# jnhansen/nd

Measured on AMD Instinct MI355X. Metric: Mpixels/s OmnibusTest dual-pol 24t x 4096 x 4096, higher is better.
Workload: dtype f32; 1 GPU; OmnibusTest C2 24t x 4096 x 4096 f32 per GPU (BASELINE configs[1]), resident in HBM; looks=9, rows_per_rank=4096

## Files before the change

### nd_amd/csrc/omnibus.hip

```cpp
#include <type_traits>

#include "omnibus_c2_device.hpp"

namespace nd_amd {

template <typename T, int PPT, bool STATS>
__global__ void __launch_bounds__(kGlobalThreads)
omnibus_c2_global_kernel(const OmniGlobalArgs<T> g, const OmniTab tab)
{
    const int tid = threadIdx.x;
    const int lane = tid & 63;
    const int64_t b = blockIdx.x;
    const int64_t row = b / g.blocks_per_row;
    const int64_t bx = b - row * g.blocks_per_row;
    const int64_t bpx0 = bx * (int64_t)(kGlobalThreads * PPT);
    const int64_t x0 = bpx0 + (int64_t)tid * PPT;
    const int k = g.k;

    if (g.write_tab && b == 0) {
        for (int j = tid; j <= k; j += kGlobalThreads) g.tab_dev[j] = tab.e[j];
    }

    {
        int64_t npx = g.nx - bpx0;
// ... 982 lines not shown
    uint32_t segd;
    const OmniTabEntry *tab;
    uint32_t *flag_idx;
    uint32_t seg;
    T *dump;
    uint32_t dump_cap;
};



__device__ __forceinline__ void store_change_row(uint8_t *res, const int k, const unsigned long long mask)
{
    if ((k & 3) == 0 && ((uintptr_t)res & 3) == 0) {
        uint32_t *w = reinterpret_cast<uint32_t *>(res);
        for (int q = 0; q < (k >> 2); ++q) {
            const unsigned nib = (unsigned)(mask >> (4 * q)) & 0xFu;
            w[q] = (nib * 0x00204081u) & 0x01010101u;
        }
    } else {
        for (int t = 0; t < k; ++t) res[t] = (uint8_t)((mask >> t) & 1ull);
    }
}

template <typename T, int KMAX>
__global__ void __launch_bounds__(64, 2) omnibus_c2_dense_kernel(const OmniDenseArgs<T> s,
                                                              const StreamScreen<32> ss)
{
    __shared__ StreamEntry tab_lds[33];
    const int lane = threadIdx.x;
    const unsigned shard = blockIdx.x % kShards;
    const unsigned lblock = blockIdx.x / kShards, nlblock = gridDim.x / kShards;
    const uint32_t n = s.flag_count[shard * kCounterStride + 1];
    if (lblock >= n) return;
    const uint32_t *list = s.dense_idx + (size_t)shard * s.segd;
    if (lane <= 32) tab_lds[lane] = ss.e[lane];
    __syncthreads();

    for (uint32_t w = lblock; w < n; w += nlblock) {
        int k = s.k;
        asm volatile("" : "+s"(k));
        const int64_t pix0 = (int64_t)(uint32_t)__builtin_amdgcn_readfirstlane((int)list[w]);
        const int64_t pix = pix0 + lane;
        const int64_t row0 = pix0 / s.nx;
        const int64_t col0 = pix0 - row0 * s.nx;
        int64_t ub;
        unsigned delta;
        bool active;
        if (s.flat) {
            active = pix < s.npix;
            ub = pix0;
            delta = (unsigned)((active ? pix : s.npix - 1) - pix0);
        } else {
            active = col0 + lane < s.nx;
            ub = row0 * s.sy + col0 * s.sx;
            delta = (unsigned)(((active ? col0 + lane : s.nx - 1) - col0) * s.sx);
        }
        T v[KMAX][4];
#pragma unroll
        for (int t = 0; t < KMAX; ++t) {
            const int64_t ot = ub + (int64_t)(t < k ? t : k - 1) * s.st;
            v[t][0] = (s.c11 + ot)[delta];
            v[t][1] = (s.c12r + ot)[delta];
            v[t][2] = (s.c12i + ot)[delta];
            v[t][3] = (s.c22 + ot)[delta];
        }
        __builtin_amdgcn_sched_barrier(0);
        unsigned mask;
        bool handoff, cand;
        dense_chain<T, KMAX, 32>(v, k, active, ss, tab_lds, mask, handoff, cand);
        if (active && !handoff && mask != 0u) store_change_row(s.change + pix * (int64_t)k, k, mask);
        if (__any(handoff)) {
            const unsigned long long m = __ballot(handoff);
            unsigned base = 0;
            if (lane == 0) base = atomicAdd(s.flag_count + shard * kCounterStride, (unsigned)__popcll(m));
            base = __shfl(base, 0);
            if (handoff) {
                const unsigned slot = base + (unsigned)__popcll(m & ((1ull << lane) - 1ull));
                s.flag_idx[(size_t)shard * s.seg + slot] = (uint32_t)pix;
                if (slot < s.dump_cap) {
                    T *d = s.dump + ((int64_t)shard * s.dump_cap + slot) * (int64_t)(4 * k);
#pragma unroll
                    for (int t = 0; t < KMAX; ++t)
                        if (t < k) {
                            Pack<T, 4> q;
                            q.v[0] = v[t][0];
                            q.v[1] = v[t][1];
                            q.v[2] = v[t][2];
                            q.v[3] = v[t][3];
// ... 1001 lines not shown
                    o.v[3] = q.d;
                    *reinterpret_cast<Pack<T, 4> *>(d + 4 * t) = o;
                }
            }
        }
    }
    if (!dense && wnp > 0) zero_fill_span(wob, wnp * k, lane);
}

template <typename T>
struct OmniSearchArgs {
    const T *c11, *c12r, *c12i, *c22;
    int64_t nx;
    int64_t sy, sx, st;
    int m11, m12, m22;
    int k;
    double nlooks, alpha;
    uint8_t *change;
    const uint32_t *flag_count, *flag_idx;
    uint32_t seg;
    const OmniTabEntry *tab;
    const T *dump;
    uint32_t dump_cap;
    unsigned long long *hand_bits;
    uint32_t hand_words;
    uint32_t *hand_count;
    uint32_t starts_max;
    uint32_t first;
};

constexpr int kScreenLong = 192;
struct DenseScreenLong {
    DenseScreenEntry e[kScreenLong + 1];
};

template <typename T, int MODE, int PXW = 64, bool FS = false, bool GSCR = false>
__global__ void __launch_bounds__(64) omnibus_c2_search_kernel(const OmniSearchArgs<T> s, const DenseScreenLong fscr)
{
    static_assert(!GSCR || (MODE == 1 && !FS), "the global-memory screen serves the double screen of MODE 1");
    constexpr bool USE_LDS = (MODE == 0);
    extern __shared__ __align__(16) unsigned char nd_smem[];
    T *lds = reinterpret_cast<T *>(nd_smem);
    const int lane = threadIdx.x;
    const int k = s.k;
    const OmniTabEntry *tabp = s.tab;
    const int kp = k + 1;
    double *scr = reinterpret_cast<double *>(nd_smem + (USE_LDS ? (size_t)k * 4 * PXW * sizeof(T) : 0));
    DenseScreenEntry *scr_f = reinterpret_cast<DenseScreenEntry *>(scr);
    if (FS) {
// ... 2 lines not shown
    } else if (!GSCR) {
        for (int j = lane; j <= k; j += 64) {
            const OmniTabEntry e = s.tab[j];
            scr[j] = e.m2rho;
            scr[kp + j] = e.pklogk;
            scr[2 * kp + j] = e.zlo_a;
            scr[3 * kp + j] = e.zhi_a;
        }
        __syncthreads();
    }
    auto screen = [&](int f, int j) -> double {
        if (GSCR) return f == 0 ? tabp[j].m2rho : (f == 1 ? tabp[j].pklogk : (f == 2 ? tabp[j].zlo_a : tabp[j].zhi_a));
        return scr[f * kp + j];
    };
    const unsigned shard = blockIdx.x % kShards;
    const unsigned lblock = blockIdx.x / kShards;
    const unsigned nlblock = gridDim.x / kShards;
    const uint32_t n = s.flag_count[shard * kCounterStride];
    const uint32_t *list = s.flag_idx + (size_t)shard * s.seg;
    if (n <= s.starts_max) return;

    for (uint32_t base = s.first + lblock * (unsigned)PXW; base < n; base += nlblock * (unsigned)PXW) {
        const uint32_t idx = base + lane;
        bool active = idx < n && lane < PXW;
        if (s.hand_bits != nullptr) {
            if (__builtin_nontemporal_load(s.hand_count) == 0u) return;
            const unsigned long long marked = s.hand_bits[(size_t)shard * s.hand_words + (base >> 6)];
            if (marked == 0ull) continue;
            active = active && ((marked >> lane) & 1ull);
        }
        const int64_t pix = active ? (int64_t)list[idx] : 0;
        const int64_t row = pix / s.nx;
        const int64_t col = pix - row * s.nx;
        const int64_t off = row * s.sy + col * s.sx;

        if (USE_LDS && (PXW == 64 || lane < PXW)) {
            if (idx < s.dump_cap) {
                const T *d = s.dump + ((int64_t)shard * s.dump_cap + idx) * (int64_t)(4 * k);
                for (int t0 = 0; t0 < k; t0 += 8) {
                    Pack<T, 4> q[8];
#pragma unroll
                    for (int u = 0; u < 8; ++u)
                        if (t0 + u < k)
                            q[u] = *reinterpret_cast<const Pack<T, 4> *>(d + 4 * (t0 + u));
#pragma unroll
                    for (int u = 0; u < 8; ++u)
                        if (t0 + u < k) {
                            const int t = t0 + u;
                            lds[(t * 4 + 0) * PXW + lane] = q[u].v[0];
                            lds[(t * 4 + 1) * PXW + lane] = q[u].v[1];
                            lds[(t * 4 + 2) * PXW + lane] = q[u].v[2];
                            lds[(t * 4 + 3) * PXW + lane] = q[u].v[3];
                        }
// ... 214 lines not shown
                        }
                    }
                }
            }
            if (!done) {
                if (fires && (k - l) >= 2) {
                    res[fire_at] = 1;
                    l = fire_at;
                    if (l >= k - 1) {
                        done = true;
                    } else {
                        A.reset();
                        fire_at = -1;
                    }
                } else {
                    done = true;
                }
            }
        }
    }
}

template <typename T>
__global__ void __launch_bounds__(64) omnibus_c2_search_starts_kernel(const OmniSearchArgs<T> s)
{
    const int lane = threadIdx.x;
    const int k = s.k;
    const int ns = k - 1;
    const int ppw = ns <= 64 ? 64 / ns : 1;
    const int nsw = ns <= 64 ? ns : 64;
    const int nsweep = ns <= 64 ? 1 : (ns <= 128 ? 2 : 3);
    const int grp = lane / nsw;
    const int l0 = lane - grp * nsw;
    const unsigned shard = blockIdx.x % kShards;
    const unsigned lblock = blockIdx.x / kShards;
    const unsigned nlblock = gridDim.x / kShards;
    const uint32_t n = s.flag_count[shard * kCounterStride];
    const bool marked_mode = s.hand_bits != nullptr;
    if (marked_mode ? (n <= s.starts_max) : (n > s.starts_max)) return;
    if (marked_mode && __builtin_nontemporal_load(s.hand_count) == 0u) return;
    const uint32_t *list = s.flag_idx + (size_t)shard * s.seg;
    const OmniTabEntry *tabp = s.tab;

    uint32_t word = lblock;
    unsigned long long todo = 0ull;
    for (uint32_t base = lblock * (uint32_t)ppw;; base += nlblock * (uint32_t)ppw) {
        uint32_t idx;
        bool active;
        if (marked_mode) {
            while (todo == 0ull && (uint64_t)word * 64u < n) {
                todo = s.hand_bits[(size_t)shard * s.hand_words + word];
                if (todo == 0ull) word += nlblock;
            }
            if (todo == 0ull) break;
            unsigned long long m = todo;
            for (int i = 0; i < grp; ++i) m &= m - 1ull;
            active = (grp < ppw) && (m != 0ull);
            idx = word * 64u + (uint32_t)(m != 0ull ? __builtin_ctzll(m) : 0);
            for (int i = 0; i < ppw; ++i) todo &= todo - 1ull;
            if (todo == 0ull) word += nlblock;
        } else {
            if (base >= n) break;
            idx = base + (uint32_t)grp;
            active = (grp < ppw) && (idx < n);
        }
        const int64_t pix = active ? (int64_t)list[idx] : 0;
        const int64_t row = pix / s.nx;
        const int64_t col = pix - row * s.nx;
        const int64_t off = row * s.sy + col * s.sx;
        const bool from_dump = active && idx < s.dump_cap;
        const T *dsrc = s.dump + ((int64_t)shard * s.dump_cap + (from_dump ? idx : 0)) * (int64_t)(4 * k);
        auto fetch = [&](int t) -> Pack<T, 4> {
            Pack<T, 4> q;
            if (from_dump) {
                q = *reinterpret_cast<const Pack<T, 4> *>(dsrc + 4 * t);
            } else {
                const int64_t o = off + (int64_t)t * s.st;
                q.v[0] = s.c11[o * s.m11];
                q.v[1] = s.c12r[o * s.m12];
                q.v[2] = s.c12i[o * s.m12];
                q.v[3] = s.c22[o * s.m22];
            }
            return q;
        };
        int nxt_a = -1, nxt_b = -1, nxt_c = -1;
        for (int sweep = 0; sweep < nsweep; ++sweep) {
        const int l = l0 + 64 * sweep;
        const bool lact = active && l < ns;
        Accum<T> A;
        A.reset();
        int fire_at = -1;
        int nxt = -1;
        auto fetch4 = [&](const int i0, Pack<T, 4> (&q)[4]) {
#pragma unroll
            for (int u = 0; u < 4; ++u) {
                const int t = l + i0 + u;
                q[u].v[0] = q[u].v[1] = q[u].v[2] = q[u].v[3] = (T)0;
                if (lact && t < k) q[u] = fetch(t);
            }
        };
        Pack<T, 4> qn[4];
        fetch4(0, qn);
        for (int i0 = 0; i0 < k; i0 += 4) {
            if (!__any(lact && l + i0 < k)) break;
            Pack<T, 4> q[4];
#pragma unroll
            for (int u = 0; u < 4; ++u) q[u] = qn[u];
            fetch4(i0 + 4, qn);
#pragma unroll
            for (int u = 0; u < 4; ++u) {
                const int i = i0 + u;
                const int t = l + i;
                const bool on = lact && t < k;
                if (on) A.step(q[u].v[0], q[u].v[1], q[u].v[2], q[u].v[3]);
                const int jj = i + 1;
                const bool last = (t == k - 1);
                const bool need = on && (jj >= 2) && (fire_at < 0 || last);
                bool fires = false, inband = false;
                if (need) {
                    const OmniTabEntry &e = tabp[jj];
                    const double za = z_approx<T>(A, jj, s.nlooks, e.m2rho, e.pklogk);
                    fires = (za > e.zhi_a) && (za < INFINITY);
                    inband = (za >= e.zlo_a) && !fires;
                }
                if (__any(inband)) {
                    if (inband) {
                        const OmniTabEntry e = tabp[jj];
                        const T zp = z_stat<T>(A, jj, s.nlooks, e);
                        const double zd = (double)zp;
                        int verdict = !(zd >= e.zlo) ? 0 : ((zd > e.zhi && zd < INFINITY) ? 1 : 2);
                        if (verdict == 2) {
                            double zv[1] = {zd}, P1[1], P2[1];
                            chisq_pair<1>(zv, 4 * (jj - 1), e.lgam, P1, P2);
                            const T P = combine_P<T>(P1[0], P2[0], e.omega2);
                            verdict = ((double)P > s.alpha) ? 1 : 0;
                        }
                        fires = (verdict == 1);
                    }
                }
                if (on && fires && fire_at < 0) fire_at = t;
                if (on && last && fires) nxt = fire_at;
            }
        }
        if (sweep == 0) nxt_a = nxt; else if (sweep == 1) nxt_b = nxt; else nxt_c = nxt;
        }
        int at = 0;
        for (int step = 0; step < ns; ++step) {
            const int ats = (at >= 0 && at < ns) ? at : 0;
            const int src = grp * nsw + (ats & 63) % nsw;
            const int na = __shfl(nxt_a, src), nb = __shfl(nxt_b, src), nc = __shfl(nxt_c, src);
            const int n1 = (ns > 64 && ats >= 128) ? nc : ((ns > 64 && ats >= 64) ? nb : na);
            if (at >= 0 && at < ns) {
                if (n1 < 0) {
                    at = -1;
                } else {
                    if (active && l0 == 0) s.change[pix * (int64_t)k + n1] = 1;
                    at = n1;
                }
            }
        }
    }
}

template <typename T, int KMAX>
__global__ void __launch_bounds__(64, 3)
omnibus_c2_search_chain_kernel(const OmniSearchArgs<T> s, const StreamScreen<32> ss)
{
    __shared__ StreamEntry tab_lds[33];
    const int lane = threadIdx.x;
    if (lane <= 32) tab_lds[lane] = ss.e[lane];
    __syncthreads();
    int k = s.k;
    asm volatile("" : "+s"(k));
    const unsigned shard = blockIdx.x % kShards;
    const unsigned lblock = blockIdx.x / kShards;
    const unsigned nlblock = gridDim.x / kShards;
    const uint32_t n = s.flag_count[shard * kCounterStride];
    if (n <= s.starts_max) return;
    const uint32_t *list = s.flag_idx + (size_t)shard * s.seg;

    for (uint32_t base = lblock * 64u; base < n; base += nlblock * 64u) {
        const uint32_t idx = base + lane;
        const bool active = idx < n;
        const int64_t pix = active ? (int64_t)list[idx] : 0;
        T v[KMAX][4];
        if (idx < s.dump_cap) {
            const T *d = s.dump + ((int64_t)shard * s.dump_cap + idx) * (int64_t)(4 * k);
#pragma unroll
            for (int t = 0; t < KMAX; ++t) {
                const Pack<T, 4> q = *reinterpret_cast<const Pack<T, 4> *>(d + 4 * (t < k ? t : k - 1));
                v[t][0] = q.v[0];
                v[t][1] = q.v[1];
                v[t][2] = q.v[2];
                v[t][3] = q.v[3];
            }
        } else {
            const int64_t row = pix / s.nx;
            const int64_t col = pix - row * s.nx;
            const int64_t off = row * s.sy + col * s.sx;
            const T *p11 = s.c11 + off * s.m11, *p12r = s.c12r + off * s.m12;
            const T *p12i = s.c12i + off * s.m12, *p22 = s.c22 + off * s.m22;
            const int64_t d11 = s.st * s.m11, d12 = s.st * s.m12, d22 = s.st * s.m22;
#pragma unroll
            for (int t = 0; t < KMAX; ++t) {
                v[t][0] = *p11;
                v[t][1] = *p12r;
                v[t][2] = *p12i;
                v[t][3] = *p22;
                if (t < k - 1) {
                    p11 += d11;
                    p12r += d12;
                    p12i += d12;
                    p22 += d22;
                }
            }
        }
        unsigned cmask;
        bool handoff, cand;
        dense_chain<T, KMAX, 32>(v, k, active, ss, tab_lds, cmask, handoff, cand);
        {
            const unsigned long long hm = __ballot(handoff);
            if (lane == 0) {
                s.hand_bits[(size_t)shard * s.hand_words + (base >> 6)] = hm;
                if (hm != 0ull) atomicAdd(s.hand_count, (unsigned)__popcll(hm));
            }
        }
        if (active && !handoff) {
            uint8_t *res = s.change + pix * (int64_t)k;
            for (int u = 1; u < k; ++u)
                if ((cmask >> u) & 1u) res[u] = 1;
        }
    }
}

std::vector<OmniTabEntry> get_table_impl(int k, uint32_t n_looks, double alpha, int dtype, int pol)
{
    static std::mutex mu;
    static std::vector<TabCacheEntry> cache;
    {
        std::lock_guard<std::mutex> lk(mu);
        for (const auto &c : cache)
            if (c.key.k == k && c.key.dtype == dtype && c.key.pol == pol && c.key.n == n_looks &&
                memcmp(&c.key.alpha, &alpha, sizeof(double)) == 0)
                return c.tab;
    }
    std::vector<OmniTabEntry> tab((size_t)k + 1);
    memset(tab.data(), 0, tab.size() * sizeof(OmniTabEntry));
    for (int j = 1; j <= k; ++j)
        tab[j] = dtype == ND_AMD_F32 ? make_entry<float>(j, n_looks, alpha, pol)
                                     : make_entry<double>(j, n_looks, alpha, pol);
    {
        std::lock_guard<std::mutex> lk(mu);
        if (cache.size() >= 32) cache.erase(cache.begin());
// ... 241 lines not shown
                          k <= (sizeof(T) == 4 ? 192 : 96) && pm_ids == nullptr && mlp == nullptr && sx == 1;
    static const bool gate_env = env_int("ND_AMD_GATE", 1) != 0;
    g.gate = flag_count + 2;
    g.gate_n = 0;
    g.gate_mode = 0;
    {
        const size_t per = (size_t)k * 4 * sizeof(T);
        size_t cap = (retain || stream_long || split_ok) ? (workspace_bytes - w.off_dump) / per / kShards : 0;
        g.seg = w.seg;
        if (cap > g.seg) cap = g.seg;
        if (split_ok) cap &= ~(size_t)63;
        g.dump = reinterpret_cast<T *>(ws + w.off_dump);
        g.dump_cap = (uint32_t)cap;
    }

    constexpr int VPPT = 16 / sizeof(T);
    const size_t es = sizeof(T);
    const bool aligned = (sx == 1) && (((uintptr_t)c11 | (uintptr_t)c12re | (uintptr_t)c12im |
                                        (uintptr_t)c22) & 15) == 0 &&
                         ((sy * (int64_t)es) % 16 == 0) && ((st * (int64_t)es) % 16 == 0);
    const bool flat = ((sx == 1) && (sy == nx)) || pm_ids != nullptr;
    g.nx = flat ? npix : nx;
    g.nrows = flat ? 1 : ny;
    unsigned long long *const hand_ws = reinterpret_cast<unsigned long long *>(ws + w.off_hand);
    const int ppt = retain ? 1 : (aligned ? VPPT : 1);
    g.blocks_per_row = ceil_div(g.nx, retain ? (int64_t)kRetainThreads : (int64_t)kGlobalThreads * ppt);
    const int64_t nblocks = g.blocks_per_row * g.nrows;
    if (nblocks > 0x7fffffffLL) {
        set_error("nd_amd_omnibus_c2: raster too large for one launch (%lld blocks)",
                  (long long)nblocks);
        return ND_AMD_EUNSUPPORTED;
    }
    auto take_sample = [&]() -> bool {
        const int64_t sblocks_total = ceil_div(npix, (int64_t)kRetainThreads);
        if (!gate_env || !retain || sblocks_total < 4096) return false;
        OmniSampleArgs<T> sa;
        sa.c11 = g.c11;
        sa.c12r = g.c12r;
        sa.c12i = g.c12i;
        sa.c22 = g.c22;
        sa.nx = g.nx;
        sa.blocks_per_row = ceil_div(g.nx, (int64_t)kRetainThreads);
        const int64_t total = sa.blocks_per_row * g.nrows;
        const int64_t nsb = pm_ids ? 128 : 512;
        sa.block_stride = total / nsb;
        sa.sy = sy;
        sa.sx = sx;
// ... 34 lines not shown
        d.tab = tab_dev;
        d.flag_idx = idx;
        d.seg = seg;
        d.dump = dump;
        d.dump_cap = dump_cap;
        int64_t per_shard_d = ceil_div(ceil_div(npix_listed, (int64_t)kShards), 64);
        if (per_shard_d > 32) per_shard_d = 32;
        if (per_shard_d < 1) per_shard_d = 1;
        const dim3 gridd((unsigned)(per_shard_d * kShards)), blockd(64);
        const DenseScreen scr = make_dense_screen<T>(htab, (int)k, n_looks);
        const StreamScreen<32> ssd = make_stream_screen<T, 32>(htab, scr, (int)k, n_looks);
        KernelTimer timer(ND_AMD_KERNEL_OMNIBUS_DENSE, sq);
        if (k <= 8)
            hipLaunchKernelGGL((omnibus_c2_dense_kernel<T, 8>), gridd, blockd, 0, sq, d, ssd);
        else if (k <= 16)
            hipLaunchKernelGGL((omnibus_c2_dense_kernel<T, 16>), gridd, blockd, 0, sq, d, ssd);
        else if (sizeof(T) == 4 && k <= 24)
            hipLaunchKernelGGL((omnibus_c2_dense_kernel<float, 24>), gridd, blockd, 0, sq,
                               reinterpret_cast<const OmniDenseArgs<float> &>(d), ssd);
        else if (sizeof(T) == 4)
            hipLaunchKernelGGL((omnibus_c2_dense_kernel<float, 32>), gridd, blockd, 0, sq,
                               reinterpret_cast<const OmniDenseArgs<float> &>(d), ssd);
    };
    const bool low_threshold = fused || stream_long || ml_chain || (pm_ids != nullptr && alpha < fused_alpha && !exact_flags);
    auto launch_search = [&](hipStream_t sq, const uint32_t *count, const uint32_t *idx, const T *dump,
                             uint32_t seg, uint32_t dump_cap, int64_t npix_listed,
                             unsigned long long *hand, uint32_t hand_words) -> int {
        OmniSearchArgs<T> s;
        s.c11 = g.c11;
        s.c12r = g.c12r;
        s.c12i = g.c12i;
        s.c22 = g.c22;
        s.nx = nx;
        s.sy = sy;
        s.sx = sx;
        s.st = st;
        s.m11 = pm_ids ? (int)pm_ids[0] : 1;
        s.m12 = pm_ids ? (int)pm_ids[1] : 1;
        s.m22 = pm_ids ? (int)pm_ids[3] : 1;
        s.k = (int)k;
        s.nlooks = g.nlooks;
        s.alpha = alpha;
        s.change = change;
        s.flag_count = count;
        s.flag_idx = idx;
        s.seg = seg;
        s.tab = tab_dev;
        s.dump = dump;
        s.dump_cap = dump_cap;
        s.hand_bits = nullptr;
        s.hand_words = hand_words;
        s.hand_count = const_cast<uint32_t *>(count) + 3;
        s.starts_max = 0;
        s.first = 0;
        const size_t scr_bytes = (size_t)(k + 1) * 4 * sizeof(double);
        const size_t lds_bytes = (size_t)k * 4 * 64 * sizeof(T) + scr_bytes;
        const bool use_lds = lds_bytes <= 150 * 1024;
        const bool fs = search_fs_enabled() && k <= kScreenLong;
        DenseScreenLong fscr;
        memset(&fscr, 0, sizeof(fscr));
        for (int j = 0; j <= kScreenLong; ++j) {
            fscr.e[j].a = -INFINITY;
            fscr.e[j].b = INFINITY;
            if (fs && j >= 1 && j <= (int)k) fscr.e[j] = make_dense_entry<T>(htab[(size_t)j], j, n_looks);
        }
        if (use_lds && lds_bytes > 64 * 1024) {
            ND_HIP_CHECK(hipFuncSetAttribute(reinterpret_cast<const void *>(&omnibus_c2_search_kernel<T, 0, 64, false>),
                                             hipFuncAttributeMaxDynamicSharedMemorySize, (int)lds_bytes));
            ND_HIP_CHECK(hipFuncSetAttribute(reinterpret_cast<const void *>(&omnibus_c2_search_kernel<T, 0, 64, true>),
                                             hipFuncAttributeMaxDynamicSharedMemorySize, (int)lds_bytes));
        }
#define ND_LAUNCH_SWEEP(MODE_, PXW_, GRID_, LDS_)                                                                  \
    do {                                                                                                          \
        if (fs)                                                                                                   \
            hipLaunchKernelGGL((omnibus_c2_search_kernel<T, MODE_, PXW_, true>), GRID_, dim3(64), LDS_, sq, s, fscr);  \
        else                                                                                                      \
            hipLaunchKernelGGL((omnibus_c2_search_kernel<T, MODE_, PXW_, false>), GRID_, dim3(64), LDS_, sq, s, fscr); \
    } while (0)
        int64_t per_shard = ceil_div(ceil_div(npix_listed, kShards), 64);
        if (per_shard > 64) per_shard = 64;
        if (per_shard < 1) per_shard = 1;
        const int64_t sblocks = per_shard * kShards;
        static const int mode_env = env_int("ND_AMD_SEARCH_MODE", -1);
        bool regs_ok = k >= 2 && k <= (sizeof(T) == 4 ? 32 : 16);
        DenseScreen scr;
        if (regs_ok) {
            scr = make_dense_screen<T>(htab, (int)k, n_looks);
            for (int j = 2; j <= (int)k; ++j)
                if (!(scr.e[j].a > -INFINITY) && !(scr.e[j].b < INFINITY)) regs_ok = false;
        }
        static const int starts_env = env_int("ND_AMD_SEARCH_STARTS", 512);
        const bool starts_form = low_threshold && k >= 2 && k <= 193 && starts_env > 0 && mode_env < 0;
        if (starts_form) {
            s.starts_max = (uint32_t)starts_env;
            KernelTimer timer(ND_AMD_KERNEL_OMNIBUS_SEARCH, sq);
            hipLaunchKernelGGL((omnibus_c2_search_starts_kernel<T>), dim3((unsigned)sblocks), dim3(64), 0, sq, s);
        }
        const bool chain_form = regs_ok && (mode_env == 3 || mode_env < 0);
        if (chain_form) {
            KernelTimer timer(ND_AMD_KERNEL_OMNIBUS_SEARCH, sq);
            s.hand_bits = hand;
            const StreamScreen<32> ss0 = make_stream_screen<T, 32>(htab, scr, (int)k, n_looks);
            const dim3 gr((unsigned)sblocks), bl(64);
            if (k <= 8)
                hipLaunchKernelGGL((omnibus_c2_search_chain_kernel<T, 8>), gr, bl, 0, sq, s, ss0);
            else if (k <= 16)
                hipLaunchKernelGGL((omnibus_c2_search_chain_kernel<T, 16>), gr, bl, 0, sq, s, ss0);
            else if (sizeof(T) == 4 && k <= 24)
                hipLaunchKernelGGL((omnibus_c2_search_chain_kernel<float, 24>), gr, bl, 0, sq,
                                   reinterpret_cast<const OmniSearchArgs<float> &>(s), ss0);
            else if (sizeof(T) == 4)
                hipLaunchKernelGGL((omnibus_c2_search_chain_kernel<float, 32>), gr, bl, 0, sq,
                                   reinterpret_cast<const OmniSearchArgs<float> &>(s), ss0);
        }
        KernelTimer timer((chain_form || starts_form) ? ND_AMD_KERNEL_OMNIBUS_EXACT : ND_AMD_KERNEL_OMNIBUS_SEARCH, sq);
        if (chain_form && k <= 65) {
            hipLaunchKernelGGL((omnibus_c2_search_starts_kernel<T>), dim3((unsigned)sblocks), dim3(64), 0, sq, s);
            return ND_AMD_OK;
        }
        const bool behind = chain_form;
        const bool from_dump = split_ok && dump_cap > 0;
        const int mode = (mode_env == 0 || mode_env == 1) ? mode_env : ((use_lds && !behind && !from_dump) ? 0 : 1);
        const int64_t xblocks = behind ? (per_shard > 16 ? 16 : per_shard) * kShards : sblocks;
        if (split_ok && dump_cap > 0) {
            if (!fs) {
                set_error("nd_amd_omnibus_c2: internal: the time-split pass A needs the float32 screen's table (k <= %d)", kScreenLong);
                return ND_AMD_EINVAL;
            }
            hipLaunchKernelGGL((omnibus_c2_search_rounds_kernel<T>), dim3((unsigned)sblocks), dim3(64), (size_t)(k + 1) * sizeof(DenseScreenEntry), sq, s, fscr);
            s.first = dump_cap;
            ND_LAUNCH_SWEEP(1, 64, dim3((unsigned)sblocks), scr_bytes);
            return ND_AMD_OK;
        }
        static const int pxw_env = env_int("ND_AMD_SEARCH_PXW", 0);
        const int pxw = pxw_env ? pxw_env : (lds_bytes > 48 * 1024 ? 16 : 64);
        if (mode == 0 && use_lds && !behind && (pxw == 32 || pxw == 16)) {
            const size_t lds_n = (size_t)k * 4 * (size_t)pxw * sizeof(T) + scr_bytes;
            int64_t ps = ceil_div(ceil_div(npix_listed, kShards), (int64_t)pxw);
            if (ps > 256) ps = 256;
            if (ps < 1) ps = 1;
            const dim3 gn((unsigned)(ps * kShards));
#define ND_LAUNCH_PXW(P)                                                                                   \
    do {                                                                                                  \
        if (lds_n > 64 * 1024) {                                                                          \
            ND_HIP_CHECK(hipFuncSetAttribute(reinterpret_cast<const void *>(&omnibus_c2_search_kernel<T, 0, P, false>), \
                                             hipFuncAttributeMaxDynamicSharedMemorySize, (int)lds_n));    \
            ND_HIP_CHECK(hipFuncSetAttribute(reinterpret_cast<const void *>(&omnibus_c2_search_kernel<T, 0, P, true>), \
                                             hipFuncAttributeMaxDynamicSharedMemorySize, (int)lds_n));    \
        }                                                                                                 \
        ND_LAUNCH_SWEEP(0, P, gn, lds_n);                                                                 \
    } while (0)
            if (pxw == 32)
                ND_LAUNCH_PXW(32);
            else
                ND_LAUNCH_PXW(16);
#undef ND_LAUNCH_PXW
            return ND_AMD_OK;
        }
        const dim3 gx((unsigned)xblocks);
        if (mode == 0 && use_lds) {
            ND_LAUNCH_SWEEP(0, 64, gx, lds_bytes);
            return ND_AMD_OK;
        }
        bool scr_lds = scr_bytes <= 64 * 1024;
        if (!scr_lds) {
            int dev = 0, lds_max = 0;
            hipError_t e = hipGetDevice(&dev);
            if (e == hipSuccess) e = hipDeviceGetAttribute(&lds_max, hipDeviceAttributeMaxSharedMemoryPerBlock, dev);
            if (e == hipSuccess && scr_bytes <= (size_t)lds_max) {
                e = hipFuncSetAttribute(reinterpret_cast<const void *>(&omnibus_c2_search_kernel<T, 1, 64, false>),
                                        hipFuncAttributeMaxDynamicSharedMemorySize, (int)scr_bytes);
                scr_lds = (e == hipSuccess);
            }
            if (e != hipSuccess) (void)hipGetLastError();
        }
        if (scr_lds)
            ND_LAUNCH_SWEEP(1, 64, gx, scr_bytes);
        else
            hipLaunchKernelGGL((omnibus_c2_search_kernel<T, 1, 64, false, true>), gx, dim3(64), 0, sq, s, fscr);
#undef ND_LAUNCH_SWEEP
        return ND_AMD_OK;
    };
// ... 386 lines not shown
            } else {
                if (kq == 16) ND_LAUNCH_SPLIT(float, 16, 8);
                else if (kq == 20) ND_LAUNCH_SPLIT(float, 20, 8);
                else ND_LAUNCH_SPLIT(float, 24, 8);
            }
        } else {
            if (k <= 32) ND_LAUNCH_SPLIT(double, 8, 4);
            else if (k <= 48) ND_LAUNCH_SPLIT(double, 12, 4);
            else if (k <= 64) ND_LAUNCH_SPLIT(double, 8, 8);
            else ND_LAUNCH_SPLIT(double, 12, 8);
        }
#undef ND_LAUNCH_SPLIT
    } else {
        KernelTimer timer(ND_AMD_KERNEL_OMNIBUS_GLOBAL, stream);
        if (retain)
            launch_retain<T>(g, tab, nblocks, stats || exact_flags, stream);
        else if (aligned)
            launch_global<T, VPPT>(g, tab, nblocks, stats || exact_flags, stream);
        else
            launch_global<T, 1>(g, tab, nblocks, stats || exact_flags, stream);
    }
    ND_HIP_CHECK(hipGetLastError());

    if (retain && g.dense_min <= 64 && (!fused || gated) && pm_ids == nullptr)
        launch_dense(stream, flag_count, flag_idx, g.dense_idx, g.dump, g.seg, g.segd, g.dump_cap, npix);
    ND_HIP_CHECK(hipGetLastError());

    {
        const int rc = launch_search(stream, flag_count, flag_idx, g.dump, g.seg, g.dump_cap, npix,
                                     hand_ws, g.seg / 64 + 1);
        if (rc != ND_AMD_OK) return rc;
    }
    ND_HIP_CHECK(hipGetLastError());
    return ND_AMD_OK;
}

}

using namespace nd_amd;

extern "C" size_t nd_amd_omnibus_c2_workspace_bytes(int dtype, int64_t ny, int64_t nx, int64_t k,
                                                    size_t *min_bytes)
{
    if (ny < 0 || nx < 0 || k < 0) return 0;
    const OmniWorkspace w = omni_layout(ny * nx, ny, k, dtype == ND_AMD_F64 ? 8 : 4);
    if (min_bytes) *min_bytes = w.min_total;
    return w.recommended;
}

extern "C" int nd_amd_omnibus_c2(const void *c11, const void *c12re, const void *c12im,
                                 const void *c22, int dtype, int64_t ny, int64_t nx, int64_t k,
                                 int64_t stride_y, int64_t stride_x, int64_t stride_t,
                                 uint32_t n_looks, double alpha, uint8_t *change, void *z_out,
// ... 123 lines not shown
```

Before: 12850 Mpixels/s.

## Fuse dense-wave pass and chain search into one work-list pass-B kernel

Merges the separate dense kernel, the chain search kernel and the follow-up starts kernel into one pass-B kernel. The fused kernel builds a prefix sum of per-shard work items (flagged-pixel chunks plus dense waves) and distributes them across blocks. Handoff pixels are resolved in place by a shared starts-search routine instead of being marked in a bitmap and picked up by another launch. The aim is to cut kernel launches, bitmap traffic and load imbalance across shards. In exchange, each block carries more code and uses more registers, which could lower occupancy.

```diff
diff --git a/nd_amd/csrc/omnibus.hip b/nd_amd/csrc/omnibus.hip
--- a/nd_amd/csrc/omnibus.hip
+++ b/nd_amd/csrc/omnibus.hip
@@ -1028,6 +1028,34 @@
     }
 }
 
+template <typename T, int KMAX, typename A>
+__device__ __forceinline__ void dense_wave_load(const A &s, const int64_t npix, const bool flat, const int k,
+                                                const int64_t pix0, const int lane, T (&v)[KMAX][4], bool &active)
+{
+    const int64_t pix = pix0 + lane;
+    const int64_t row0 = pix0 / s.nx;
+    const int64_t col0 = pix0 - row0 * s.nx;
+    int64_t ub;
+    unsigned delta;
+    if (flat) {
+        active = pix < npix;
+        ub = pix0;
+        delta = (unsigned)((active ? pix : npix - 1) - pix0);
+    } else {
+        active = col0 + lane < s.nx;
+        ub = row0 * s.sy + col0 * s.sx;
+        delta = (unsigned)(((active ? col0 + lane : s.nx - 1) - col0) * s.sx);
+    }
+#pragma unroll
+    for (int t = 0; t < KMAX; ++t) {
+        const int64_t ot = ub + (int64_t)(t < k ? t : k - 1) * s.st;
+        v[t][0] = (s.c11 + ot)[delta];
+        v[t][1] = (s.c12r + ot)[delta];
+        v[t][2] = (s.c12i + ot)[delta];
+        v[t][3] = (s.c22 + ot)[delta];
+    }
+}
+
 template <typename T, int KMAX>
 __global__ void __launch_bounds__(64, 2) omnibus_c2_dense_kernel(const OmniDenseArgs<T> s,
                                                               const StreamScreen<32> ss)
@@ -1047,29 +1075,9 @@
         asm volatile("" : "+s"(k));
         const int64_t pix0 = (int64_t)(uint32_t)__builtin_amdgcn_readfirstlane((int)list[w]);
         const int64_t pix = pix0 + lane;
-        const int64_t row0 = pix0 / s.nx;
-        const int64_t col0 = pix0 - row0 * s.nx;
-        int64_t ub;
-        unsigned delta;
         bool active;
-        if (s.flat) {
-            active = pix < s.npix;
-            ub = pix0;
-            delta = (unsigned)((active ? pix : s.npix - 1) - pix0);
-        } else {
-            active = col0 + lane < s.nx;
-            ub = row0 * s.sy + col0 * s.sx;
-            delta = (unsigned)(((active ? col0 + lane : s.nx - 1) - col0) * s.sx);
-        }
         T v[KMAX][4];
-#pragma unroll
-        for (int t = 0; t < KMAX; ++t) {
-            const int64_t ot = ub + (int64_t)(t < k ? t : k - 1) * s.st;
-            v[t][0] = (s.c11 + ot)[delta];
-            v[t][1] = (s.c12r + ot)[delta];
-            v[t][2] = (s.c12i + ot)[delta];
-            v[t][3] = (s.c22 + ot)[delta];
-        }
+        dense_wave_load<T, KMAX>(s, s.npix, s.flat != 0, k, pix0, lane, v, active);
         __builtin_amdgcn_sched_barrier(0);
         unsigned mask;
         bool handoff, cand;
@@ -2117,9 +2125,6 @@
     const OmniTabEntry *tab;
     const T *dump;
     uint32_t dump_cap;
-    unsigned long long *hand_bits;
-    uint32_t hand_words;
-    uint32_t *hand_count;
     uint32_t starts_max;
     uint32_t first;
 };
@@ -2168,13 +2173,7 @@
 
     for (uint32_t base = s.first + lblock * (unsigned)PXW; base < n; base += nlblock * (unsigned)PXW) {
         const uint32_t idx = base + lane;
-        bool active = idx < n && lane < PXW;
-        if (s.hand_bits != nullptr) {
-            if (__builtin_nontemporal_load(s.hand_count) == 0u) return;
-            const unsigned long long marked = s.hand_bits[(size_t)shard * s.hand_words + (base >> 6)];
-            if (marked == 0ull) continue;
-            active = active && ((marked >> lane) & 1ull);
-        }
+        const bool active = idx < n && lane < PXW;
         const int64_t pix = active ? (int64_t)list[idx] : 0;
         const int64_t row = pix / s.nx;
         const int64_t col = pix - row * s.nx;
@@ -2435,213 +2434,265 @@
 }
 
 template <typename T>
+__device__ __forceinline__ void search_starts_pixels(const OmniSearchArgs<T> &s, const int k, const int lane,
+                                                     const bool active, const int64_t pix, const bool from_dump,
+                                                     const T *dsrc)
+{
+    const int ns = k - 1;
+    const int nsw = ns <= 64 ? ns : 64;
+    const int nsweep = ns <= 64 ? 1 : (ns <= 128 ? 2 : 3);
+    const int grp = lane / nsw;
+    const int l0 = lane - grp * nsw;
+    const OmniTabEntry *tabp = s.tab;
+    const int64_t row = pix / s.nx;
+    const int64_t col = pix - row * s.nx;
+    const int64_t off = row * s.sy + col * s.sx;
+    auto fetch = [&](int t) -> Pack<T, 4> {
+        Pack<T, 4> q;
+        if (from_dump) {
+            q = *reinterpret_cast<const Pack<T, 4> *>(dsrc + 4 * t);
+        } else {
+            const int64_t o = off + (int64_t)t * s.st;
+            q.v[0] = s.c11[o * s.m11];
+            q.v[1] = s.c12r[o * s.m12];
+            q.v[2] = s.c12i[o * s.m12];
+            q.v[3] = s.c22[o * s.m22];
+        }
+        return q;
+    };
+    int nxt_a = -1, nxt_b = -1, nxt_c = -1;
+    for (int sweep = 0; sweep < nsweep; ++sweep) {
+    const int l = l0 + 64 * sweep;
+    const bool lact = active && l < ns;
+    Accum<T> A;
+    A.reset();
+    int fire_at = -1;
+    int nxt = -1;
+    auto fetch4 = [&](const int i0, Pack<T, 4> (&q)[4]) {
+#pragma unroll
+        for (int u = 0; u < 4; ++u) {
+            const int t = l + i0 + u;
+            q[u].v[0] = q[u].v[1] = q[u].v[2] = q[u].v[3] = (T)0;
+            if (lact && t < k) q[u] = fetch(t);
+        }
+    };
+    Pack<T, 4> qn[4];
+    fetch4(0, qn);
+    for (int i0 = 0; i0 < k; i0 += 4) {
+        if (!__any(lact && l + i0 < k)) break;
+        Pack<T, 4> q[4];
+#pragma unroll
+        for (int u = 0; u < 4; ++u) q[u] = qn[u];
+        fetch4(i0 + 4, qn);
+#pragma unroll
+        for (int u = 0; u < 4; ++u) {
+            const int i = i0 + u;
+            const int t = l + i;
+            const bool on = lact && t < k;
+            if (on) A.step(q[u].v[0], q[u].v[1], q[u].v[2], q[u].v[3]);
+            const int jj = i + 1;
+            const bool last = (t == k - 1);
+            const bool need = on && (jj >= 2) && (fire_at < 0 || last);
+            bool fires = false, inband = false;
+            if (need) {
+                const OmniTabEntry &e = tabp[jj];
+                const double za = z_approx<T>(A, jj, s.nlooks, e.m2rho, e.pklogk);
+                fires = (za > e.zhi_a) && (za < INFINITY);
+                inband = (za >= e.zlo_a) && !fires;
+            }
+            if (__any(inband)) {
+                if (inband) {
+                    const OmniTabEntry e = tabp[jj];
+                    const T zp = z_stat<T>(A, jj, s.nlooks, e);
+                    const double zd = (double)zp;
+                    int verdict = !(zd >= e.zlo) ? 0 : ((zd > e.zhi && zd < INFINITY) ? 1 : 2);
+                    if (verdict == 2) {
+                        double zv[1] = {zd}, P1[1], P2[1];
+                        chisq_pair<1>(zv, 4 * (jj - 1), e.lgam, P1, P2);
+                        const T P = combine_P<T>(P1[0], P2[0], e.omega2);
+                        verdict = ((double)P > s.alpha) ? 1 : 0;
+                    }
+                    fires = (verdict == 1);
+                }
+            }
+            if (on && fires && fire_at < 0) fire_at = t;
+            if (on && last && fires) nxt = fire_at;
+        }
+    }
+    if (sweep == 0) nxt_a = nxt; else if (sweep == 1) nxt_b = nxt; else nxt_c = nxt;
+    }
+    int at = 0;
+    for (int step = 0; step < ns; ++step) {
+        const int ats = (at >= 0 && at < ns) ? at : 0;
+        const int src = grp * nsw + (ats & 63) % nsw;
+        const int na = __shfl(nxt_a, src), nb = __shfl(nxt_b, src), nc = __shfl(nxt_c, src);
+        const int n1 = (ns > 64 && ats >= 128) ? nc : ((ns > 64 && ats >= 64) ? nb : na);
+        if (at >= 0 && at < ns) {
+            if (n1 < 0) {
+                at = -1;
+            } else {
+                if (active && l0 == 0) s.change[pix * (int64_t)k + n1] = 1;
+                at = n1;
+            }
+        }
+    }
+}
+
+template <typename T>
 __global__ void __launch_bounds__(64) omnibus_c2_search_starts_kernel(const OmniSearchArgs<T> s)
 {
     const int lane = threadIdx.x;
     const int k = s.k;
     const int ns = k - 1;
     const int ppw = ns <= 64 ? 64 / ns : 1;
-    const int nsw = ns <= 64 ? ns : 64;
-    const int nsweep = ns <= 64 ? 1 : (ns <= 128 ? 2 : 3);
-    const int grp = lane / nsw;
-    const int l0 = lane - grp * nsw;
+    const int grp = lane / (ns <= 64 ? ns : 64);
     const unsigned shard = blockIdx.x % kShards;
     const unsigned lblock = blockIdx.x / kShards;
     const unsigned nlblock = gridDim.x / kShards;
     const uint32_t n = s.flag_count[shard * kCounterStride];
-    const bool marked_mode = s.hand_bits != nullptr;
-    if (marked_mode ? (n <= s.starts_max) : (n > s.starts_max)) return;
-    if (marked_mode && __builtin_nontemporal_load(s.hand_count) == 0u) return;
+    if (n > s.starts_max) return;
     const uint32_t *list = s.flag_idx + (size_t)shard * s.seg;
-    const OmniTabEntry *tabp = s.tab;
-
-    uint32_t word = lblock;
-    unsigned long long todo = 0ull;
-    for (uint32_t base = lblock * (uint32_t)ppw;; base += nlblock * (uint32_t)ppw) {
-        uint32_t idx;
-        bool active;
-        if (marked_mode) {
-            while (todo == 0ull && (uint64_t)word * 64u < n) {
-                todo = s.hand_bits[(size_t)shard * s.hand_words + word];
-                if (todo == 0ull) word += nlblock;
-            }
-            if (todo == 0ull) break;
-            unsigned long long m = todo;
-            for (int i = 0; i < grp; ++i) m &= m - 1ull;
-            active = (grp < ppw) && (m != 0ull);
-            idx = word * 64u + (uint32_t)(m != 0ull ? __builtin_ctzll(m) : 0);
-            for (int i = 0; i < ppw; ++i) todo &= todo - 1ull;
-            if (todo == 0ull) word += nlblock;
-        } else {
-            if (base >= n) break;
-            idx = base + (uint32_t)grp;
-            active = (grp < ppw) && (idx < n);
-        }
+    for (uint32_t base = lblock * (uint32_t)ppw; base < n; base += nlblock * (uint32_t)ppw) {
+        const uint32_t idx = base + (uint32_t)grp;
+        const bool active = (grp < ppw) && (idx < n);
         const int64_t pix = active ? (int64_t)list[idx] : 0;
-        const int64_t row = pix / s.nx;
-        const int64_t col = pix - row * s.nx;
-        const int64_t off = row * s.sy + col * s.sx;
         const bool from_dump = active && idx < s.dump_cap;
         const T *dsrc = s.dump + ((int64_t)shard * s.dump_cap + (from_dump ? idx : 0)) * (int64_t)(4 * k);
-        auto fetch = [&](int t) -> Pack<T, 4> {
-            Pack<T, 4> q;
-            if (from_dump) {
-                q = *reinterpret_cast<const Pack<T, 4> *>(dsrc + 4 * t);
-            } else {
-                const int64_t o = off + (int64_t)t * s.st;
-                q.v[0] = s.c11[o * s.m11];
-                q.v[1] = s.c12r[o * s.m12];
-                q.v[2] = s.c12i[o * s.m12];
-                q.v[3] = s.c22[o * s.m22];
-            }
-            return q;
-        };
-        int nxt_a = -1, nxt_b = -1, nxt_c = -1;
-        for (int sweep = 0; sweep < nsweep; ++sweep) {
-        const int l = l0 + 64 * sweep;
-        const bool lact = active && l < ns;
-        Accum<T> A;
-        A.reset();
-        int fire_at = -1;
-        int nxt = -1;
-        auto fetch4 = [&](const int i0, Pack<T, 4> (&q)[4]) {
-#pragma unroll
-            for (int u = 0; u < 4; ++u) {
-                const int t = l + i0 + u;
-                q[u].v[0] = q[u].v[1] = q[u].v[2] = q[u].v[3] = (T)0;
-                if (lact && t < k) q[u] = fetch(t);
-            }
-        };
-        Pack<T, 4> qn[4];
-        fetch4(0, qn);
-        for (int i0 = 0; i0 < k; i0 += 4) {
-            if (!__any(lact && l + i0 < k)) break;
-            Pack<T, 4> q[4];
-#pragma unroll
-            for (int u = 0; u < 4; ++u) q[u] = qn[u];
-            fetch4(i0 + 4, qn);
-#pragma unroll
-            for (int u = 0; u < 4; ++u) {
-                const int i = i0 + u;
-                const int t = l + i;
-                const bool on = lact && t < k;
-                if (on) A.step(q[u].v[0], q[u].v[1], q[u].v[2], q[u].v[3]);
-                const int jj = i + 1;
-                const bool last = (t == k - 1);
-                const bool need = on && (jj >= 2) && (fire_at < 0 || last);
-                bool fires = false, inband = false;
-                if (need) {
-                    const OmniTabEntry &e = tabp[jj];
-                    const double za = z_approx<T>(A, jj, s.nlooks, e.m2rho, e.pklogk);
-                    fires = (za > e.zhi_a) && (za < INFINITY);
-                    inband = (za >= e.zlo_a) && !fires;
-                }
-                if (__any(inband)) {
-                    if (inband) {
-                        const OmniTabEntry e = tabp[jj];
-                        const T zp = z_stat<T>(A, jj, s.nlooks, e);
-                        const double zd = (double)zp;
-                        int verdict = !(zd >= e.zlo) ? 0 : ((zd > e.zhi && zd < INFINITY) ? 1 : 2);
-                        if (verdict == 2) {
-                            double zv[1] = {zd}, P1[1], P2[1];
-                            chisq_pair<1>(zv, 4 * (jj - 1), e.lgam, P1, P2);
-                            const T P = combine_P<T>(P1[0], P2[0], e.omega2);
-                            verdict = ((double)P > s.alpha) ? 1 : 0;
-                        }
-                        fires = (verdict == 1);
-                    }
-                }
-                if (on && fires && fire_at < 0) fire_at = t;
-                if (on && last && fires) nxt = fire_at;
-            }
-        }
-        if (sweep == 0) nxt_a = nxt; else if (sweep == 1) nxt_b = nxt; else nxt_c = nxt;
-        }
-        int at = 0;
-        for (int step = 0; step < ns; ++step) {
-            const int ats = (at >= 0 && at < ns) ? at : 0;
-            const int src = grp * nsw + (ats & 63) % nsw;
-            const int na = __shfl(nxt_a, src), nb = __shfl(nxt_b, src), nc = __shfl(nxt_c, src);
-            const int n1 = (ns > 64 && ats >= 128) ? nc : ((ns > 64 && ats >= 64) ? nb : na);
-            if (at >= 0 && at < ns) {
-                if (n1 < 0) {
-                    at = -1;
-                } else {
-                    if (active && l0 == 0) s.change[pix * (int64_t)k + n1] = 1;
-                    at = n1;
-                }
-            }
-        }
+        search_starts_pixels<T>(s, k, lane, active, pix, from_dump, dsrc);
     }
 }
 
+struct OmniPassbDense {
+    const uint32_t *dense_idx;
+    uint32_t segd;
+    int flat;
+    int64_t npix;
+};
+
+constexpr int passb_waves(const int kmax, const size_t elem) { return (elem == 4 && kmax <= 16) ? 3 : 2; }
+
 template <typename T, int KMAX>
-__global__ void __launch_bounds__(64, 3)
-omnibus_c2_search_chain_kernel(const OmniSearchArgs<T> s, const StreamScreen<32> ss)
+__global__ void __launch_bounds__(64, passb_waves(KMAX, sizeof(T)))
+omnibus_c2_passb_kernel(const OmniSearchArgs<T> s, const OmniPassbDense dn, const StreamScreen<32> ss)
 {
     __shared__ StreamEntry tab_lds[33];
+    __shared__ uint32_t item_end[kShards];
+    __shared__ uint32_t list_n[kShards];
+    static_assert(kShards == 128, "two shards per lane");
     const int lane = threadIdx.x;
+    uint32_t nl[2], ni[2];
+#pragma unroll
+    for (int h = 0; h < 2; ++h) {
+        const uint32_t *cnt = s.flag_count + (size_t)(lane + 64 * h) * kCounterStride;
+        uint32_t n = cnt[0];
+        if (n <= s.starts_max) n = 0;
+        nl[h] = n;
+        ni[h] = ((n + 63u) >> 6) + (dn.dense_idx != nullptr ? cnt[1] : 0u);
+    }
+#pragma unroll
+    for (int d = 1; d < 64; d <<= 1) {
+        const uint32_t u0 = __shfl_up(ni[0], d), u1 = __shfl_up(ni[1], d);
+        if (lane >= d) {
+            ni[0] += u0;
+            ni[1] += u1;
+        }
+    }
+    ni[1] += __shfl(ni[0], 63);
+    const uint32_t total = __shfl(ni[1], 63);
+    if (blockIdx.x >= total) return;
     if (lane <= 32) tab_lds[lane] = ss.e[lane];
+    item_end[lane] = ni[0];
+    item_end[lane + 64] = ni[1];
+    list_n[lane] = nl[0];
+    list_n[lane + 64] = nl[1];
     __syncthreads();
-    int k = s.k;
-    asm volatile("" : "+s"(k));
-    const unsigned shard = blockIdx.x % kShards;
-    const unsigned lblock = blockIdx.x / kShards;
-    const unsigned nlblock = gridDim.x / kShards;
-    const uint32_t n = s.flag_count[shard * kCounterStride];
-    if (n <= s.starts_max) return;
-    const uint32_t *list = s.flag_idx + (size_t)shard * s.seg;
-
-    for (uint32_t base = lblock * 64u; base < n; base += nlblock * 64u) {
-        const uint32_t idx = base + lane;
-        const bool active = idx < n;
-        const int64_t pix = active ? (int64_t)list[idx] : 0;
+
+    for (uint32_t item = blockIdx.x; item < total; item += gridDim.x) {
+        int k = s.k;
+        asm volatile("" : "+s"(k));
+        const unsigned shard = (unsigned)__popcll(__ballot(item_end[lane] <= item)) +
+                               (unsigned)__popcll(__ballot(item_end[lane + 64] <= item));
+        const uint32_t first = shard ? (uint32_t)__builtin_amdgcn_readfirstlane((int)item_end[shard - 1]) : 0u;
+        const uint32_t n = (uint32_t)__builtin_amdgcn_readfirstlane((int)list_n[shard]);
+        const uint32_t local = item - first;
+        const bool chunk = local < ((n + 63u) >> 6);
+        uint32_t base = 0;
+        uint32_t pixl = 0;
+        bool active;
         T v[KMAX][4];
-        if (idx < s.dump_cap) {
-            const T *d = s.dump + ((int64_t)shard * s.dump_cap + idx) * (int64_t)(4 * k);
-#pragma unroll
-            for (int t = 0; t < KMAX; ++t) {
-                const Pack<T, 4> q = *reinterpret_cast<const Pack<T, 4> *>(d + 4 * (t < k ? t : k - 1));
-                v[t][0] = q.v[0];
-                v[t][1] = q.v[1];
-                v[t][2] = q.v[2];
-                v[t][3] = q.v[3];
+        if (chunk) {
+            base = local * 64u;
+            const uint32_t idx = base + lane;
+            active = idx < n;
+            pixl = active ? s.flag_idx[(size_t)shard * s.seg + idx] : 0u;
+            if (idx < s.dump_cap) {
+                const T *d = s.dump + ((int64_t)shard * s.dump_cap + idx) * (int64_t)(4 * k);
+#pragma unroll
+                for (int t = 0; t < KMAX; ++t) {
+                    const Pack<T, 4> q = *reinterpret_cast<const Pack<T, 4> *>(d + 4 * (t < k ? t : k - 1));
+                    v[t][0] = q.v[0];
+                    v[t][1] = q.v[1];
+                    v[t][2] = q.v[2];
+                    v[t][3] = q.v[3];
+                }
+            } else {
+                const int64_t pix = (int64_t)pixl;
+                const int64_t row = pix / s.nx;
+                const int64_t col = pix - row * s.nx;
+                const int64_t off = row * s.sy + col * s.sx;
+                const T *p11 = s.c11 + off * s.m11, *p12r = s.c12r + off * s.m12;
+                const T *p12i = s.c12i + off * s.m12, *p22 = s.c22 + off * s.m22;
+                const int64_t d11 = s.st * s.m11, d12 = s.st * s.m12, d22 = s.st * s.m22;
+#pragma unroll
+                for (int t = 0; t < KMAX; ++t) {
+                    v[t][0] = *p11;
+                    v[t][1] = *p12r;
+                    v[t][2] = *p12i;
+                    v[t][3] = *p22;
+                    if (t < k - 1) {
+                        p11 += d11;
+                        p12r += d12;
+                        p12i += d12;
+                        p22 += d22;
+                    }
+                }
             }
         } else {
-            const int64_t row = pix / s.nx;
-            const int64_t col = pix - row * s.nx;
-            const int64_t off = row * s.sy + col * s.sx;
-            const T *p11 = s.c11 + off * s.m11, *p12r = s.c12r + off * s.m12;
-            const T *p12i = s.c12i + off * s.m12, *p22 = s.c22 + off * s.m22;
-            const int64_t d11 = s.st * s.m11, d12 = s.st * s.m12, d22 = s.st * s.m22;
-#pragma unroll
-            for (int t = 0; t < KMAX; ++t) {
-                v[t][0] = *p11;
-                v[t][1] = *p12r;
-                v[t][2] = *p12i;
-                v[t][3] = *p22;
-                if (t < k - 1) {
-                    p11 += d11;
-                    p12r += d12;
-                    p12i += d12;
-                    p22 += d22;
-                }
-            }
-        }
+            const uint32_t w = local - ((n + 63u) >> 6);
+            const uint32_t pix0 = (uint32_t)__builtin_amdgcn_readfirstlane((int)dn.dense_idx[(size_t)shard * dn.segd + w]);
+            dense_wave_load<T, KMAX>(s, dn.npix, dn.flat != 0, k, (int64_t)pix0, lane, v, active);
+            pixl = pix0 + (uint32_t)lane;
+        }
+        __builtin_amdgcn_sched_barrier(0);
         unsigned cmask;
         bool handoff, cand;
         dense_chain<T, KMAX, 32>(v, k, active, ss, tab_lds, cmask, handoff, cand);
-        {
-            const unsigned long long hm = __ballot(handoff);
-            if (lane == 0) {
-                s.hand_bits[(size_t)shard * s.hand_words + (base >> 6)] = hm;
-                if (hm != 0ull) atomicAdd(s.hand_count, (unsigned)__popcll(hm));
-            }
-        }
         if (active && !handoff) {
-            uint8_t *res = s.change + pix * (int64_t)k;
-            for (int u = 1; u < k; ++u)
-                if ((cmask >> u) & 1u) res[u] = 1;
+            uint8_t *res = s.change + (int64_t)pixl * (int64_t)k;
+            if (chunk) {
+                for (int u = 1; u < k; ++u)
+                    if ((cmask >> u) & 1u) res[u] = 1;
+            } else if (cmask != 0u) {
+                store_change_row(res, k, cmask);
+            }
+        }
+        unsigned long long todo = __ballot(handoff);
+        if (todo != 0ull) {
+            const int ns = k - 1;
+            const int ppw = 64 / ns;
+            const int grp = lane / ns;
+            do {
+                unsigned long long m = todo;
+                for (int i = 0; i < grp; ++i) m &= m - 1ull;
+                const bool act = (grp < ppw) && (m != 0ull);
+                const int src = m != 0ull ? __builtin_ctzll(m) : 0;
+                const int64_t pix = (int64_t)(uint32_t)__shfl((int)pixl, src);
+                const uint32_t idx = base + (uint32_t)src;
+                const bool from_dump = chunk && act && idx < s.dump_cap;
+                const T *dsrc = s.dump + ((int64_t)shard * s.dump_cap + (from_dump ? idx : 0)) * (int64_t)(4 * k);
+                search_starts_pixels<T>(s, k, lane, act, act ? pix : 0, from_dump, dsrc);
+                for (int i = 0; i < ppw; ++i) todo &= todo - 1ull;
+            } while (todo != 0ull);
         }
     }
 }
@@ -2929,7 +2980,6 @@
     const bool flat = ((sx == 1) && (sy == nx)) || pm_ids != nullptr;
     g.nx = flat ? npix : nx;
     g.nrows = flat ? 1 : ny;
-    unsigned long long *const hand_ws = reinterpret_cast<unsigned long long *>(ws + w.off_hand);
     const int ppt = retain ? 1 : (aligned ? VPPT : 1);
     g.blocks_per_row = ceil_div(g.nx, retain ? (int64_t)kRetainThreads : (int64_t)kGlobalThreads * ppt);
     const int64_t nblocks = g.blocks_per_row * g.nrows;
@@ -3010,10 +3060,19 @@
             hipLaunchKernelGGL((omnibus_c2_dense_kernel<float, 32>), gridd, blockd, 0, sq,
                                reinterpret_cast<const OmniDenseArgs<float> &>(d), ssd);
     };
+    static const int mode_env = env_int("ND_AMD_SEARCH_MODE", -1);
+    bool regs_ok = k >= 2 && k <= (sizeof(T) == 4 ? 32 : 16);
+    DenseScreen scr_b;
+    if (regs_ok) {
+        scr_b = make_dense_screen<T>(htab, (int)k, n_looks);
+        for (int j = 2; j <= (int)k; ++j)
+            if (!(scr_b.e[j].a > -INFINITY) && !(scr_b.e[j].b < INFINITY)) regs_ok = false;
+    }
+    const bool chain_form = regs_ok && (mode_env == 3 || mode_env < 0);
     const bool low_threshold = fused || stream_long || ml_chain || (pm_ids != nullptr && alpha < fused_alpha && !exact_flags);
     auto launch_search = [&](hipStream_t sq, const uint32_t *count, const uint32_t *idx, const T *dump,
                              uint32_t seg, uint32_t dump_cap, int64_t npix_listed,
-                             unsigned long long *hand, uint32_t hand_words) -> int {
+                             const uint32_t *dense_idx, uint32_t segd) -> int {
         OmniSearchArgs<T> s;
         s.c11 = g.c11;
         s.c12r = g.c12r;
@@ -3036,9 +3095,6 @@
         s.tab = tab_dev;
         s.dump = dump;
         s.dump_cap = dump_cap;
-        s.hand_bits = nullptr;
-        s.hand_words = hand_words;
-        s.hand_count = const_cast<uint32_t *>(count) + 3;
         s.starts_max = 0;
         s.first = 0;
         const size_t scr_bytes = (size_t)(k + 1) * 4 * sizeof(double);
@@ -3069,14 +3125,6 @@
         if (per_shard > 64) per_shard = 64;
         if (per_shard < 1) per_shard = 1;
         const int64_t sblocks = per_shard * kShards;
-        static const int mode_env = env_int("ND_AMD_SEARCH_MODE", -1);
-        bool regs_ok = k >= 2 && k <= (sizeof(T) == 4 ? 32 : 16);
-        DenseScreen scr;
-        if (regs_ok) {
-            scr = make_dense_screen<T>(htab, (int)k, n_looks);
-            for (int j = 2; j <= (int)k; ++j)
-                if (!(scr.e[j].a > -INFINITY) && !(scr.e[j].b < INFINITY)) regs_ok = false;
-        }
         static const int starts_env = env_int("ND_AMD_SEARCH_STARTS", 512);
         const bool starts_form = low_threshold && k >= 2 && k <= 193 && starts_env > 0 && mode_env < 0;
         if (starts_form) {
@@ -3084,32 +3132,30 @@
             KernelTimer timer(ND_AMD_KERNEL_OMNIBUS_SEARCH, sq);
             hipLaunchKernelGGL((omnibus_c2_search_starts_kernel<T>), dim3((unsigned)sblocks), dim3(64), 0, sq, s);
         }
-        const bool chain_form = regs_ok && (mode_env == 3 || mode_env < 0);
         if (chain_form) {
             KernelTimer timer(ND_AMD_KERNEL_OMNIBUS_SEARCH, sq);
-            s.hand_bits = hand;
-            const StreamScreen<32> ss0 = make_stream_screen<T, 32>(htab, scr, (int)k, n_looks);
+            OmniPassbDense dn;
+            dn.dense_idx = dense_idx;
+            dn.segd = segd;
+            dn.flat = flat ? 1 : 0;
+            dn.npix = npix;
+            const StreamScreen<32> ss0 = make_stream_screen<T, 32>(htab, scr_b, (int)k, n_looks);
             const dim3 gr((unsigned)sblocks), bl(64);
             if (k <= 8)
-                hipLaunchKernelGGL((omnibus_c2_search_chain_kernel<T, 8>), gr, bl, 0, sq, s, ss0);
+                hipLaunchKernelGGL((omnibus_c2_passb_kernel<T, 8>), gr, bl, 0, sq, s, dn, ss0);
             else if (k <= 16)
-                hipLaunchKernelGGL((omnibus_c2_search_chain_kernel<T, 16>), gr, bl, 0, sq, s, ss0);
+                hipLaunchKernelGGL((omnibus_c2_passb_kernel<T, 16>), gr, bl, 0, sq, s, dn, ss0);
             else if (sizeof(T) == 4 && k <= 24)
-                hipLaunchKernelGGL((omnibus_c2_search_chain_kernel<float, 24>), gr, bl, 0, sq,
-                                   reinterpret_cast<const OmniSearchArgs<float> &>(s), ss0);
+                hipLaunchKernelGGL((omnibus_c2_passb_kernel<float, 24>), gr, bl, 0, sq,
+                                   reinterpret_cast<const OmniSearchArgs<float> &>(s), dn, ss0);
             else if (sizeof(T) == 4)
-                hipLaunchKernelGGL((omnibus_c2_search_chain_kernel<float, 32>), gr, bl, 0, sq,
-                                   reinterpret_cast<const OmniSearchArgs<float> &>(s), ss0);
-        }
-        KernelTimer timer((chain_form || starts_form) ? ND_AMD_KERNEL_OMNIBUS_EXACT : ND_AMD_KERNEL_OMNIBUS_SEARCH, sq);
-        if (chain_form && k <= 65) {
-            hipLaunchKernelGGL((omnibus_c2_search_starts_kernel<T>), dim3((unsigned)sblocks), dim3(64), 0, sq, s);
+                hipLaunchKernelGGL((omnibus_c2_passb_kernel<float, 32>), gr, bl, 0, sq,
+                                   reinterpret_cast<const OmniSearchArgs<float> &>(s), dn, ss0);
             return ND_AMD_OK;
         }
-        const bool behind = chain_form;
+        KernelTimer timer(starts_form ? ND_AMD_KERNEL_OMNIBUS_EXACT : ND_AMD_KERNEL_OMNIBUS_SEARCH, sq);
         const bool from_dump = split_ok && dump_cap > 0;
-        const int mode = (mode_env == 0 || mode_env == 1) ? mode_env : ((use_lds && !behind && !from_dump) ? 0 : 1);
-        const int64_t xblocks = behind ? (per_shard > 16 ? 16 : per_shard) * kShards : sblocks;
+        const int mode = (mode_env == 0 || mode_env == 1) ? mode_env : ((use_lds && !from_dump) ? 0 : 1);
         if (split_ok && dump_cap > 0) {
             if (!fs) {
                 set_error("nd_amd_omnibus_c2: internal: the time-split pass A needs the float32 screen's table (k <= %d)", kScreenLong);
@@ -3122,7 +3168,7 @@
         }
         static const int pxw_env = env_int("ND_AMD_SEARCH_PXW", 0);
         const int pxw = pxw_env ? pxw_env : (lds_bytes > 48 * 1024 ? 16 : 64);
-        if (mode == 0 && use_lds && !behind && (pxw == 32 || pxw == 16)) {
+        if (mode == 0 && use_lds && (pxw == 32 || pxw == 16)) {
             const size_t lds_n = (size_t)k * 4 * (size_t)pxw * sizeof(T) + scr_bytes;
             int64_t ps = ceil_div(ceil_div(npix_listed, kShards), (int64_t)pxw);
             if (ps > 256) ps = 256;
@@ -3145,7 +3191,7 @@
 #undef ND_LAUNCH_PXW
             return ND_AMD_OK;
         }
-        const dim3 gx((unsigned)xblocks);
+        const dim3 gx((unsigned)sblocks);
         if (mode == 0 && use_lds) {
             ND_LAUNCH_SWEEP(0, 64, gx, lds_bytes);
             return ND_AMD_OK;
@@ -3578,13 +3624,15 @@
     }
     ND_HIP_CHECK(hipGetLastError());
 
-    if (retain && g.dense_min <= 64 && (!fused || gated) && pm_ids == nullptr)
+    const bool dense_waves = retain && g.dense_min <= 64 && (!fused || gated) && pm_ids == nullptr;
+    if (dense_waves && !chain_form) {
         launch_dense(stream, flag_count, flag_idx, g.dense_idx, g.dump, g.seg, g.segd, g.dump_cap, npix);
-    ND_HIP_CHECK(hipGetLastError());
+        ND_HIP_CHECK(hipGetLastError());
+    }
 
     {
         const int rc = launch_search(stream, flag_count, flag_idx, g.dump, g.seg, g.dump_cap, npix,
-                                     hand_ws, g.seg / 64 + 1);
+                                     dense_waves && chain_form ? g.dense_idx : nullptr, g.segd);
         if (rc != ND_AMD_OK) return rc;
     }
     ND_HIP_CHECK(hipGetLastError());
```

After: 12950 Mpixels/s, median of 6. About the same (+0.8%).
